# NVlabs/CenterPose

Measured on NVIDIA H100. Metric: images/sec at 512x512 DLA-34 (dla_34 + DCNv2, 7 heads, decode + PnP), higher is better.
Workload: dtype tf32x3

## Files before the change

### centerpose_b200/csrc/common.cuh

```cuda
#pragma once
#include <cuda_runtime.h>
#include <stdint.h>
#include <stdio.h>
#include <string>

#include "../../include/centerpose_b200.h"

namespace cp {

void set_error(const std::string& msg);
int fail(int code, const std::string& msg);
extern thread_local long long g_launch_counter;

#define CP_CUDA_CHECK(expr)                                                              \
  do {                                                                                   \
    cudaError_t _e = (expr);                                                             \
    if (_e != cudaSuccess)                                                               \
      return ::cp::fail(CP_ERR_CUDA, std::string(#expr) + ": " + cudaGetErrorString(_e)); \
  } while (0)

#define CP_LAUNCH_CHECK(what)                                                            \
  do {                                                                                   \
    cudaError_t _e = cudaGetLastError();                                                 \
    if (_e != cudaSuccess)                                                               \
// ... 16 lines not shown
  int srcStride[4];
  int nsrc;
  int B, Hin, Win, Cin;
  int Hout, Wout, Cout, CoutPad;
  int kh, kw, stride, pad;
  int Kpad;
  const float* wgt;
  const float* bias;
  const float* residual;
  int resStride;
  int relu;
  int res_after_relu;
  float* out;
  int outStride;
  int out_nchw;
  const float* offmask;
  int omStride;
  int mask_is_logit;
  int mode;
  const void* wgt_umma;
  float* splitk_ws;
  size_t splitk_ws_floats;
  int fuse_n, fuse_hidden;
  const float* fuse_w[16];
  const float* fuse_b[16];
  float* fuse_out[16];
  int fuse_cout[16];
  int ipm;
  long long wstride, tstride;
  unsigned nchw_per_model;
};
inline int model_ipm(const IgemmParams& p) { return p.ipm > 0 ? p.ipm : p.B; }

int launch_igemm_fp32(const IgemmParams& p, cudaStream_t stream);

int decode_pnp_models(const cp_decode_params* prm, int models, const cp_heads* heads, const double* meta, float* dets,
                      float* poses, int32_t* n_valid, void* workspace, size_t workspace_bytes, void* stream);

struct LaunchInfo {
  int BN = 0;
  int ksplit = 1;
  long long grid = 0;
};

bool conv3_c16_supported(const IgemmParams& p);
int launch_conv3_c16(const IgemmParams& p, cudaStream_t stream);
bool stem_supported(const IgemmParams& p);
// ... 129 lines not shown
```

### centerpose_b200/csrc/conv_tma.cu

```cuda
#include <cuda.h>

#include "common.cuh"
#include "umma_common.cuh"

namespace cp {
namespace {

constexpr int TM_BM = 128;
constexpr int TM_THREADS = 384;
constexpr int TM_THREADS_X3 = 512;

struct TmaConvParams {
  CUtensorMap amap[4];
  int nsrc;
  int srcC[4];
  int B, H, W, Cin, Cout, CoutPad, BN;
  int k;
  int tile_m;
  int Wt, boxh;
  int tiles_per_image;
  long long total_tiles;
  long long m_tiles;
  uint32_t slab_bytes, slab_stride;
  int SA, SB;
  const float* bias;
  const float* residual;
  int resStride, relu, res_after_relu;
  float* out;
  int outStride, out_nchw;
  int round_tf32;
  int cslab;
  int x3;
  int group;
  const unsigned char* wtiles;
  int ksplit, sps;
  float* part;
  int fuse, tph;
  const float* fuse_w[16];
  const float* fuse_b[16];
  float* fuse_out[16];
  int fuse_cout[16];
  int ipm;
  long long wstride, tstride, tiles_per_model;
};

using namespace umma;

struct TmaCtl {
  unsigned long long a_full[4], a_empty[4], a_split[4];
  unsigned long long b_full[8], b_empty[8];
};
static_assert(sizeof(TmaCtl) <= 512, "control block");

struct TileGeo {
  int n_tile, img, g0, r_lo, model;
  long long pos0;
};
template <bool MULTI>
__device__ __forceinline__ TileGeo decode_tile(const TmaConvParams& p, long long ct, int n_tiles) {
  TileGeo g;
  g.n_tile = (int)(ct % n_tiles);
// ... 20 lines not shown

template <bool MULTI>
__device__ __forceinline__ bool tile_position(const TmaConvParams& p, const TileGeo& g, int i, int* n, int* oy, int* ox, int* m) {
  bool valid;
  if (p.k == 3) {
    const int gg = g.g0 + i;
    *oy = gg / p.Wt;
    const int xp = gg - *oy * p.Wt;
    *ox = xp - 1;
    *n = g.img;
    valid = (*oy < p.H) && (xp >= 1) && (xp <= p.W);
  } else {
    const long long pix = g.pos0 + i;
    valid = pix < (MULTI ? (long long)(g.model + 1) * p.ipm : (long long)p.B) * p.H * p.W;
    const long long pp = valid ? pix : 0;
    *ox = (int)(pp % p.W);
    const long long t = pp / p.W;
    *oy = (int)(t % p.H);
    *n = (int)(t / p.H);
  }
  *m = (int)(((size_t)*n * p.H + *oy) * p.W + *ox);
  return valid;
}

template <bool X3, bool FUSE, int BN, bool MULTI>
__global__ void __launch_bounds__(X3 ? TM_THREADS_X3 : TM_THREADS, 1) conv_tma_kernel(const __grid_constant__ TmaConvParams p) {
  extern __shared__ __align__(1024) unsigned char smem[];
  TmaCtl* ctl = reinterpret_cast<TmaCtl*>(smem);
  if (threadIdx.x == 0) griddep_launch_dependents();
  const uint32_t slabs0 = (smem_u32(smem) + 512u + 1023u) & ~1023u;
  const uint32_t rowb = (uint32_t)p.cslab * 4u;
  const uint32_t btile_bytes = (uint32_t)BN * rowb * (X3 ? 2u : 1u);
  const uint32_t a_stage = p.slab_stride * (X3 ? 2u : 1u);
  const uint32_t btiles0 = slabs0 + (uint32_t)p.SA * a_stage;
  const uint32_t drain0 = btiles0 + (uint32_t)p.SB * btile_bytes;

  const int tid = threadIdx.x, warp = tid >> 5, lane = tid & 31;
  const int n_tiles = p.CoutPad / BN;
  const int taps = p.k * p.k;
  const int KS_SPLIT = p.ksplit;
  const int sps = p.sps;
  const int KB = sps * taps;
  const int KB_all = (p.Cin / p.cslab) * taps;
  const long long total_tiles = p.total_tiles;
  const long long tph = FUSE ? p.tph : 1;
  auto tile_at = [&](long long it) { return ((long long)blockIdx.x + (it / tph) * gridDim.x) * tph + (it % tph); };
// ... 28 lines not shown
              cb += p.srcC[src];
              ++src;
            }
            mbar_wait(smem_u32(&ctl->a_empty[stage]), phase ^ 1u);
            const uint32_t bar = smem_u32(&ctl->a_full[stage]);
            mbar_arrive_expect_tx(bar, p.slab_bytes);
            const uint32_t dst = slabs0 + (uint32_t)stage * a_stage;
            if (p.k == 3)
              tma_load_4d(dst, &p.amap[src], s * p.cslab - cb, -1, g.r_lo - 1, g.img, bar);
            else
              tma_load_2d(dst, &p.amap[src], s * p.cslab - cb, (int)g.pos0, bar);
            if (++stage == p.SA) {
              stage = 0;
              phase ^= 1u;
            }
          }
        }
      }
      __syncwarp();
    } else if (warp == 1) {
      if (lane == 0) {
        int stage = 0;
        uint32_t phase = 0;
        for (long long it = 0, tile = tile_at(0); tile < total_tiles; tile = tile_at(++it)) {
          const unsigned char* wsrc;
          if constexpr (MULTI) {
            const TileGeo g = decode_tile<MULTI>(p, tile / KS_SPLIT, n_tiles);
            wsrc = p.wtiles + (size_t)g.model * p.tstride +
                   ((size_t)g.n_tile * KB_all + (size_t)(tile % KS_SPLIT) * KB) * btile_bytes;
          } else {
            const int n_tile = (int)((tile / KS_SPLIT) % n_tiles);
            wsrc = p.wtiles + ((size_t)n_tile * KB_all + (size_t)(tile % KS_SPLIT) * KB) * btile_bytes;
          }
          for (int kb = 0; kb < KB; ++kb) {
            mbar_wait(smem_u32(&ctl->b_empty[stage]), phase ^ 1u);
            const uint32_t bar = smem_u32(&ctl->b_full[stage]);
            mbar_arrive_expect_tx(bar, btile_bytes);
            bulk_g2s(btiles0 + (uint32_t)stage * btile_bytes, wsrc + (size_t)kb * btile_bytes, btile_bytes, bar);
            if (++stage == p.SB) {
              stage = 0;
              phase ^= 1u;
            }
          }
        }
      }
      __syncwarp();
    }
  } else if (X3 && warp >= 12) {
    asm volatile("setmaxnreg.dec.sync.aligned.u32 48;");
    const int st = tid - 384;
    int stage = 0;
    uint32_t phase = 0;
    const uint32_t nchunk = p.slab_bytes >> 4;
    for (long long it = 0, tile = tile_at(0); tile < total_tiles; tile = tile_at(++it)) {
      for (int s = 0; s < sps; ++s) {
        mbar_wait(smem_u32(&ctl->a_full[stage]), phase);
        const uint32_t hi = slabs0 + (uint32_t)stage * a_stage;
        const uint32_t lo = hi + p.slab_stride;
        for (uint32_t c0 = st; c0 < nchunk; c0 += 128 * 4) {
          float4 v[4];
#pragma unroll
// ... 26 lines not shown
    float* dstage = reinterpret_cast<float*>(smem + (drain0 - smem_u32(smem))) + (size_t)c * (DRAIN_STAGE_BYTES / 4);
    const uint32_t bar_a = smem_u32(X3 ? &ctl->a_split[0] : &ctl->a_full[0]);
    const uint32_t bar_a_empty = smem_u32(&ctl->a_empty[0]);
    const uint32_t bar_b_full = smem_u32(&ctl->b_full[0]), bar_b_empty = smem_u32(&ctl->b_empty[0]);
    const uint32_t a_lo_u = p.slab_stride >> 4, b_lo_u = ((uint32_t)BN * rowb) >> 4;
    EpiParams ep;
    ep.bias = p.bias;
    ep.residual = p.residual;
    ep.resStride = p.resStride;
    ep.relu = p.relu;
    ep.res_after_relu = p.res_after_relu;
    ep.round_tf32 = p.round_tf32;
    ep.out = p.out;
    ep.outStride = p.outStride;
    ep.out_nchw = p.out_nchw;
    ep.Cout = p.Cout;
    ep.CoutPad = p.CoutPad;
    ep.H = p.H;
    ep.W = p.W;
    int sa = 0, sb = 0;
    uint32_t pa = 0, pb = 0;
    float acc[BN / 2];
    float sums[X3 ? BN / 2 : 1];
    float acc2[FUSE ? 16 : 1];
#pragma unroll
    for (int j = 0; j < BN / 2; ++j) acc[j] = 0.f;
#pragma unroll
    for (int j = 0; j < (FUSE ? 16 : 1); ++j) acc2[j] = 0.f;
    for (long long it = 0, tile = tile_at(0); tile < total_tiles; tile = tile_at(++it)) {
      const TileGeo g = decode_tile<MULTI>(p, tile / KS_SPLIT, n_tiles);
      const uint32_t row0 = (p.k == 3 ? (uint32_t)(g.g0 - 1 - g.r_lo * p.Wt) : 0u) + (uint32_t)c * 64u;
#pragma unroll
      for (int j = 0; j < (X3 ? BN / 2 : 1); ++j) sums[j] = 0.f;
      const int group = X3 ? p.group : 1;
      const bool overlap = X3 && p.SA > 1;
      int tap = 0;
      auto release_prev = [&]() {
        if (wt == 0) {
          mbar_arrive(bar_b_empty + 8u * (uint32_t)(sb == 0 ? p.SB - 1 : sb - 1));
          if (tap == 0) mbar_arrive(bar_a_empty + 8u * (uint32_t)(sa == 0 ? p.SA - 1 : sa - 1));
        }
      };
      for (int kb0 = 0; kb0 < KB; kb0 += group) {
        const int n_kb = min(group, KB - kb0);
        for (int i = 0; i < n_kb; ++i) {
          if (tap == 0) mbar_wait(bar_a + 8u * (uint32_t)sa, pa);
          const int ky = tap / 3, kx = tap - ky * 3;
          const uint32_t arow = row0 + (p.k == 3 ? (uint32_t)(ky * p.Wt + kx) : 0u);
          mbar_wait(bar_b_full + 8u * (uint32_t)sb, pb);
          const uint64_t da = make_desc(slabs0 + (uint32_t)sa * a_stage + arow * rowb, p.cslab);
          const uint64_t db = make_desc(btiles0 + (uint32_t)sb * btile_bytes, p.cslab);
// ... 12 lines not shown
          }
          if (++tap == taps) {
            tap = 0;
            if (++sa == p.SA) {
              sa = 0;
              pa ^= 1u;
            }
          }
          if (!overlap) {
            wg_wait<0>();
            release_prev();
          }
        }
        wg_wait<0>();
        if (overlap) release_prev();
#pragma unroll
        for (int j = 0; j < (X3 ? BN / 2 : 1); ++j)
          if (X3) sums[j] += acc[X3 ? j : 0];
      }
      if (X3) {
#pragma unroll
        for (int j = 0; j < BN / 2; ++j) acc[j] = 0.f;
      }
      const int r_me = wt >> 1;
      int n, oy, ox, m;
      const bool valid = tile_position<MULTI>(p, g, c * 64 + r_me, &n, &oy, &ox, &m);
      const int col_end = min(p.Cout, (g.n_tile + 1) * BN);
      const int head = FUSE ? g.n_tile / p.tph : 0, part = FUSE ? g.n_tile - head * p.tph : 0;
      const size_t wofs = MULTI ? (size_t)g.model * p.wstride : 0;
      if (MULTI) ep.bias = p.bias + wofs;
      if (FUSE && part == 0) {
#pragma unroll
        for (int j = 0; j < (FUSE ? 16 : 1); ++j) acc2[j] = 0.f;
      }
      auto fn = [&](int r, int cb, float (&v)[16]) {
        if (cb >= BN) return;
        if (!FUSE && KS_SPLIT > 1) {
          const long long mn = tile / KS_SPLIT;
          const int ks = (int)(tile % KS_SPLIT);
          float4* mine = reinterpret_cast<float4*>(p.part) + (((size_t)mn * KS_SPLIT + ks) * (BN >> 2) + (cb >> 2)) * p.tile_m +
                         c * 64 + r;
#pragma unroll
          for (int q = 0; q < 4; ++q) __stcg(mine + (size_t)q * p.tile_m, make_float4(v[4 * q], v[4 * q + 1], v[4 * q + 2], v[4 * q + 3]));
        } else if (FUSE) {
          const float* b1 = p.bias + wofs + (size_t)g.n_tile * BN + cb;
          const float4* w2 = reinterpret_cast<const float4*>(p.fuse_w[head] + wofs) + ((size_t)part * BN + cb) * 4;
#pragma unroll
          for (int q = 0; q < 16; ++q) {
            const float h = fmaxf(v[q] + __ldg(b1 + q), 0.f);
#pragma unroll
            for (int u = 0; u < 4; ++u) {
              const float4 w = __ldg(w2 + q * 4 + u);
              acc2[FUSE ? 4 * u + 0 : 0] = fmaf(h, w.x, acc2[FUSE ? 4 * u + 0 : 0]);
              acc2[FUSE ? 4 * u + 1 : 0] = fmaf(h, w.y, acc2[FUSE ? 4 * u + 1 : 0]);
              acc2[FUSE ? 4 * u + 2 : 0] = fmaf(h, w.z, acc2[FUSE ? 4 * u + 2 : 0]);
              acc2[FUSE ? 4 * u + 3 : 0] = fmaf(h, w.w, acc2[FUSE ? 4 * u + 3 : 0]);
            }
          }
        } else {
          epilogue_row<16>(ep, v, valid, m, n, oy, ox, g.n_tile * BN + cb, col_end);
        }
      };
      if constexpr (X3 && FUSE) {
        const int rg = wt >> 3, hh = (wt >> 2) & 1, og = wt & 3;
        const int fr0 = (wt >> 5) * 16 + ((wt & 31) >> 2), fcq = (wt & 3) * 2;
        const float* b1 = p.bias + wofs + (size_t)g.n_tile * BN;
        const float4* w2 = reinterpret_cast<const float4*>(p.fuse_w[head] + wofs) + (size_t)part * BN * 4 + og;
        auto at = [&](int r, int col) { return r * 32 + ((((col >> 2) ^ r) & 7) << 2) + (col & 3); };
#pragma unroll
        for (int c0 = 0; c0 < BN; c0 += 32) {
#pragma unroll
          for (int j = 0; j < BN / 8; ++j) {
            if (j * 8 >= c0 && j * 8 < c0 + 32) {
              const int col = j * 8 - c0 + fcq;
              const float bx = __ldg(b1 + c0 + col), by = __ldg(b1 + c0 + col + 1);
              dstage[at(fr0, col)] = fmaxf(sums[X3 ? 4 * j : 0] + bx, 0.f);
              dstage[at(fr0, col + 1)] = fmaxf(sums[X3 ? 4 * j + 1 : 0] + by, 0.f);
              dstage[at(fr0 + 8, col)] = fmaxf(sums[X3 ? 4 * j + 2 : 0] + bx, 0.f);
              dstage[at(fr0 + 8, col + 1)] = fmaxf(sums[X3 ? 4 * j + 3 : 0] + by, 0.f);
            }
          }
          wg_bar_sync(1 + c);
#pragma unroll
          for (int m4 = 0; m4 < 4; ++m4) {
            const int k0 = 16 * hh + 4 * m4;
            float4 hv[4];
#pragma unroll
            for (int i = 0; i < 4; ++i) hv[i] = *reinterpret_cast<const float4*>(dstage + at(rg + 16 * i, k0));
#pragma unroll
            for (int kk = 0; kk < 4; ++kk) {
              const float4 w = __ldg(w2 + (size_t)(c0 + k0 + kk) * 4);
#pragma unroll
              for (int i = 0; i < 4; ++i) {
                const float h = kk == 0 ? hv[i].x : kk == 1 ? hv[i].y : kk == 2 ? hv[i].z : hv[i].w;
                acc2[FUSE ? 4 * i + 0 : 0] = fmaf(h, w.x, acc2[FUSE ? 4 * i + 0 : 0]);
                acc2[FUSE ? 4 * i + 1 : 0] = fmaf(h, w.y, acc2[FUSE ? 4 * i + 1 : 0]);
                acc2[FUSE ? 4 * i + 2 : 0] = fmaf(h, w.z, acc2[FUSE ? 4 * i + 2 : 0]);
                acc2[FUSE ? 4 * i + 3 : 0] = fmaf(h, w.w, acc2[FUSE ? 4 * i + 3 : 0]);
              }
            }
          }
          wg_bar_sync(1 + c);
        }
        if (part == p.tph - 1) {
#pragma unroll
          for (int j = 0; j < 16; ++j) acc2[FUSE ? j : 0] += __shfl_xor_sync(0xffffffffu, acc2[FUSE ? j : 0], 4);
          if (hh == 0) {
            const int co = p.fuse_cout[head];
            const size_t plane = (size_t)p.H * p.W;
#pragma unroll
            for (int i = 0; i < 4; ++i) {
              int n1, oy1, ox1, m1;
              if (!tile_position<MULTI>(p, g, c * 64 + rg + 16 * i, &n1, &oy1, &ox1, &m1)) continue;
              float* o = p.fuse_out[head] + ((size_t)n1 * co * p.H + oy1) * p.W + ox1;
#pragma unroll
              for (int u = 0; u < 4; ++u)
                if (4 * og + u < co) o[(4 * og + u) * plane] = acc2[FUSE ? 4 * i + u : 0] + __ldg(p.fuse_b[head] + wofs + 4 * og + u);
            }
          }
        }
        continue;
      }
      if constexpr (X3)
        drain_rows<BN>(sums, dstage, wt, 1 + c, fn);
      else
        drain_rows<BN>(acc, dstage, wt, 1 + c, fn);
      if (FUSE && part == p.tph - 1) {
#pragma unroll
        for (int j = 0; j < (FUSE ? 16 : 1); ++j) acc2[j] += __shfl_xor_sync(0xffffffffu, acc2[j], 1);
        if ((wt & 1) == 0 && valid) {
          const int co = p.fuse_cout[head];
          float* o = p.fuse_out[head] + ((size_t)n * co * p.H + oy) * p.W + ox;
          const size_t plane = (size_t)p.H * p.W;
#pragma unroll
          for (int j = 0; j < 16; ++j)
            if (j < co) o[j * plane] = acc2[FUSE ? j : 0] + __ldg(p.fuse_b[head] + wofs + j);
        }
      }
    }
  }
}

__global__ void pack_tma_weight_kernel(const float* __restrict__ src, int ld, int Cin, int taps, int Cout, int BN, int n_tiles,
                                       int round_tf32, int x3, int cslab, unsigned char* __restrict__ dst) {
  const int KB = (Cin / cslab) * taps;
  const int cpr = cslab / 4;
  const size_t rowb = (size_t)cslab * 4;
  const size_t total = (size_t)n_tiles * KB * BN * cpr;
  for (size_t i = blockIdx.x * (size_t)blockDim.x + threadIdx.x; i < total; i += (size_t)gridDim.x * blockDim.x) {
    const int q = i % cpr;
    size_t t = i / cpr;
    const int nr = t % BN;
    t /= BN;
    const int kb = t % KB;
    const int nt = t / KB;
    const int n = nt * BN + nr;
    const int slab = kb / taps, tap = kb - slab * taps;
    float v[4];
#pragma unroll
    for (int j = 0; j < 4; ++j) {
      const int k = tap * Cin + slab * cslab + q * 4 + j;
// ... 143 lines not shown
      cuuint32_t box[4] = {(cuuint32_t)cs, (cuuint32_t)Wt, (cuuint32_t)boxh, 1};
      cuuint32_t es[4] = {1, 1, 1, 1};
      r = enc(&maps[s], CU_TENSOR_MAP_DATA_TYPE_FLOAT32, 4, (void*)p.src[s], dims, strides, box, es,
              CU_TENSOR_MAP_INTERLEAVE_NONE, swz, CU_TENSOR_MAP_L2_PROMOTION_L2_256B,
              CU_TENSOR_MAP_FLOAT_OOB_FILL_NONE);
    } else {
      cuuint64_t dims[2] = {(cuuint64_t)p.srcC[s], (cuuint64_t)Bmax * p.Hin * p.Win};
      cuuint64_t strides[1] = {(cuuint64_t)p.srcStride[s] * 4};
      cuuint32_t box[2] = {(cuuint32_t)cs, (cuuint32_t)TM_BM};
      cuuint32_t es[2] = {1, 1};
      r = enc(&maps[s], CU_TENSOR_MAP_DATA_TYPE_FLOAT32, 2, (void*)p.src[s], dims, strides, box, es,
              CU_TENSOR_MAP_INTERLEAVE_NONE, swz, CU_TENSOR_MAP_L2_PROMOTION_L2_256B,
              CU_TENSOR_MAP_FLOAT_OOB_FILL_NONE);
    }
    if (r != CUDA_SUCCESS) return fail(CP_ERR_CUDA, "cuTensorMapEncodeTiled failed with code " + std::to_string((int)r));
  }
  return CP_OK;
}

template <bool X3, bool FUSE, bool MULTI>
static int launch_conv_tma_kernel(const TmaConvParams& q, const cudaLaunchConfig_t& cfg0) {
  void (*kern)(TmaConvParams) = nullptr;
  switch (q.BN) {
    case 16: kern = conv_tma_kernel<X3, FUSE, 16, MULTI>; break;
    case 32: kern = conv_tma_kernel<X3, FUSE, 32, MULTI>; break;
    case 64: kern = conv_tma_kernel<X3, FUSE, 64, MULTI>; break;
    case 128: kern = conv_tma_kernel<X3, FUSE, 128, MULTI>; break;
    default: return fail(CP_ERR_INVALID, "conv_tma: unsupported N tile");
  }
  static PerDevice<bool, 4> configured;
  const int slot = q.BN == 128 ? 3 : (q.BN == 64 ? 2 : (q.BN == 32 ? 1 : 0));
  if (!configured.here(slot)) {
    CP_CUDA_CHECK(cudaFuncSetAttribute(kern, cudaFuncAttributeMaxDynamicSharedMemorySize, 227 * 1024));
    configured.here(slot) = true;
  }
  cudaLaunchConfig_t cfg = cfg0;
  cudaLaunchAttribute attr[1];
  attr[0].id = cudaLaunchAttributeProgrammaticStreamSerialization;
  attr[0].val.programmaticStreamSerializationAllowed = 1;
  cfg.attrs = attr;
  cfg.numAttrs = g_pdl ? 1 : 0;
  CP_CUDA_CHECK(cudaLaunchKernelEx(&cfg, kern, q));
  CP_LAUNCH_CHECK("conv_tma_kernel");
  return CP_OK;
}

int launch_conv_tma(const IgemmParams& p, const void* maps, const ConvKernel& k, cudaStream_t stream, LaunchInfo* info) {
  if (!p.wgt_umma) return fail(CP_ERR_INVALID, "conv_tma: weight tiles missing");
  if (p.B % model_ipm(p)) return fail(CP_ERR_INVALID, "conv_tma: batch is not a whole number of models");
  const bool x3 = k.x3;
  TmaConvParams q;
  memset(&q, 0, sizeof(q));
// ... 24 lines not shown
    q.slab_bytes = (uint32_t)q.boxh * q.Wt * (uint32_t)q.cslab * 4u;
  } else {
    q.tiles_per_image = 0;
    q.tiles_per_model = ((long long)q.ipm * p.Hin * p.Win + q.tile_m - 1) / q.tile_m;
    m_tiles = (size_t)q.tiles_per_model * (p.B / q.ipm);
    q.slab_bytes = (uint32_t)q.tile_m * (uint32_t)q.cslab * 4u;
  }
  q.slab_stride = (q.slab_bytes + 1023u) & ~1023u;
  const uint32_t btile = (uint32_t)q.BN * (uint32_t)q.cslab * 4u * (x3 ? 2u : 1u);
  const uint32_t a_stage = q.slab_stride * (x3 ? 2u : 1u);
  size_t smem = 0;
  if (int rc = tma_smem_layout(a_stage, btile, q.k, &q.SA, &q.SB, &smem)) return rc;
  q.bias = p.bias;
  q.residual = p.residual;
  q.resStride = p.resStride;
  q.relu = p.relu;
  q.res_after_relu = p.res_after_relu;
  q.out = p.out;
  q.outStride = p.outStride;
  q.out_nchw = p.out_nchw;
  q.round_tf32 = k.round_out;
  q.wtiles = (const unsigned char*)p.wgt_umma;
  if (p.fuse_n > 0) {
    if (p.fuse_hidden % q.BN || p.CoutPad != p.fuse_n * p.fuse_hidden || !p.relu || p.residual || (x3 && q.BN != 128))
      return fail(CP_ERR_INVALID, "conv_tma: fused 1x1 needs relu, no residual and head_conv a multiple of the N tile");
    q.fuse = 1;
    q.tph = p.fuse_hidden / q.BN;
    for (int h = 0; h < p.fuse_n; ++h) {
      q.fuse_w[h] = p.fuse_w[h];
      q.fuse_b[h] = p.fuse_b[h];
      q.fuse_out[h] = p.fuse_out[h];
      q.fuse_cout[h] = p.fuse_cout[h];
    }
  }
  q.m_tiles = (long long)m_tiles;
  q.part = p.splitk_ws;
  const long long mn = (long long)m_tiles * (p.CoutPad / q.BN);
  const int nslab = q.Cin / q.cslab;
  int num_sms = 0;
  if (int rc = device_sm_count(&num_sms)) return rc;
  q.ksplit = x3 && !q.fuse ? splitk_factor(mn, nslab, num_sms, (size_t)q.tile_m * q.BN, p.splitk_ws_floats) : 1;
  q.sps = nslab / q.ksplit;
  q.total_tiles = mn * q.ksplit;
  if (q.total_tiles >= (1ll << 31)) return fail(CP_ERR_INVALID, "conv_tma: too many tiles");
  cudaLaunchConfig_t cfg{};
  cfg.gridDim = dim3((unsigned)(q.total_tiles < num_sms ? q.total_tiles : num_sms));
  cfg.blockDim = dim3(x3 ? TM_THREADS_X3 : TM_THREADS);
  cfg.dynamicSmemBytes = smem;
  cfg.stream = stream;
  const bool multi = p.B > q.ipm;
  int rc;
  if (multi)
// ... 22 lines not shown
```

### centerpose_b200/csrc/plan.cu

```cuda
#include <stdlib.h>
#include <string.h>

#include <map>
#include <memory>
#include <set>
#include <string>
#include <vector>

#include "arena_pack.h"
#include "common.cuh"

namespace cp {

thread_local std::string g_last_error;
void set_error(const std::string& msg) { g_last_error = msg; }
thread_local long long g_launch_counter = 0;
thread_local int g_pdl = 0;

int fail(int code, const std::string& msg) {
  g_last_error = msg;
  return code;
}

namespace {
// ... 74 lines not shown

}
}

using namespace cp;

struct cp_plan {
  cp_config cfg;
  std::vector<std::string> head_names;
  int B = 0, H = 0, W = 0;
  std::vector<Op> ops;
  std::vector<PackJob> jobs;
  float* act = nullptr;
  size_t act_floats = 0;
  float* wts = nullptr;
  size_t w_floats = 0;
  std::vector<Act> head_bufs;
  bool loaded = false;
  int launches = 0;
  void* decode_ws = nullptr;
  size_t decode_ws_bytes = 0;
  double* gn_stats = nullptr;
  bool no_dcn_tma = false;
  unsigned char* umma_wts = nullptr;
  size_t umma_bytes = 0;
  float* splitk_ws = nullptr;
  int models = 1;
  std::vector<char> model_loaded;
  unsigned ext_per_model = 0;
  bool reuse = false;
  std::vector<ArenaAlloc> bufs;
  std::vector<size_t> buf_off;
};

namespace cp {
namespace {

struct Builder {
  cp_plan* P;
  size_t act_cur = 0, w_cur = 0;
  int B;

  size_t walloc(size_t n) {
    size_t o = w_cur;
    w_cur += (n + 63) / 64 * 64;
    return o;
// ... 458 lines not shown
  p.residual = op.has_res ? P->act + op.res.off : nullptr;
  p.resStride = op.res.stride;
  p.relu = op.relu;
  p.res_after_relu = op.res_after_relu;
  if (op.out_head >= 0) {
    p.out = head_out ? head_out[op.out_head] : nullptr;
    p.out_nchw = 1;
    p.outStride = 0;
  } else {
    p.out = P->act + op.out.off;
    p.outStride = op.out.stride;
  }
  if (op.mode == IGEMM_DCN) {
    p.offmask = P->act + op.om.off;
    p.omStride = op.om.stride;
    p.mask_is_logit = 1;
  }
  p.mode = op.mode;
  if (op.fuse_heads) {
    p.fuse_n = (int)op.head_children.size();
    p.fuse_hidden = P->cfg.head_conv;
    for (int i = 0; i < p.fuse_n; ++i) {
      const Op& ch = P->ops[op.head_children[i]];
      p.fuse_w[i] = P->wts + ch.w_off;
      p.fuse_b[i] = P->wts + ch.b_off;
      p.fuse_out[i] = head_out ? head_out[ch.out_head] : nullptr;
      p.fuse_cout[i] = ch.Cout;
    }
  }
}

void plan_params(const cp_plan* P, const Op& op, IgemmParams* p) {
  static const float* const no_ext[4] = {};
  igemm_params(P, op, P->B, no_ext, nullptr, p);
}

void select_kernels(cp_plan* P) {
  const ConvPolicy pol{true, !P->no_dcn_tma, true, true};
  static const float residual_present = 0.f;
  P->umma_bytes = 0;
  for (auto& op : P->ops) {
    if (op.type != OP_IGEMM) continue;
    IgemmParams p;
    plan_params(P, op, &p);
    if (op.has_res) p.residual = &residual_present;
    op.kernel = select_conv_kernel(p, P->cfg.precision, pol);
    op.tile_off = P->umma_bytes;
    P->umma_bytes += (op.kernel.wbytes + 1023) / 1024 * 1024;
  }
  const int head_conv = P->cfg.head_conv;
  for (auto& op : P->ops) {
    if (op.head_children.empty() || op.kernel.family != CP_FAM_CONV_TMA) continue;
    const int bn = op.kernel.BN;
    bool ok = op.relu && !op.has_res && (head_conv % bn == 0) && (int)op.head_children.size() <= 16 &&
              op.CoutPad == (int)op.head_children.size() * head_conv && (!op.kernel.x3 || bn == 128);
    for (int ci : op.head_children) {
      const Op& ch = P->ops[ci];
      ok = ok && ch.CoutPad == 16 && ch.w_ld == 16 && ch.Cin == head_conv && ch.out_head >= 0 && !ch.relu && !ch.has_res;
    }
    if (!ok) continue;
    op.fuse_heads = true;
    for (int ci : op.head_children) P->ops[ci].fused_away = true;
  }
}

template <class F>
void for_each_act(cp_plan* P, Op& op, F f) {
  if (op.fused_away) return;
  switch (op.type) {
    case OP_IGEMM:
      for (int s = 0; s < op.nsrc; ++s) f(op.src[s]);
      if (op.has_res) f(op.res);
      if (op.mode == IGEMM_DCN) f(op.om);
      if (op.out_head >= 0) f(P->head_bufs[op.out_head]);
      else if (!op.fuse_heads) f(op.out);
      if (op.fuse_heads)
        for (int c : op.head_children) f(P->head_bufs[P->ops[c].out_head]);
      return;
    case OP_MAXPOOL:
    case OP_MAXPOOL3:
    case OP_UPADD:
// ... 105 lines not shown
  if (cfg->height % 32 || cfg->width % 32 || cfg->height <= 0 || cfg->width <= 0)
    return fail(CP_ERR_INVALID, "cp_plan_create: height/width must be positive multiples of 32");
  if (cfg->max_batch <= 0 || cfg->num_heads <= 0 || cfg->num_heads > CP_MAX_HEADS)
    return fail(CP_ERR_INVALID, "cp_plan_create: bad batch / head count");
  if (cfg->head_conv <= 0 || cfg->head_conv % 64)
    return fail(CP_ERR_INVALID, "cp_plan_create: head_conv must be a positive multiple of 64");
  if (cfg->arch == CP_ARCH_DLAV1_34 && cfg->head_conv != 256)
    return fail(CP_ERR_INVALID, "cp_plan_create: dlav1 GroupNorm path needs head_conv == 256");
  P->cfg = *cfg;
  for (int i = 0; i < cfg->num_heads; ++i) {
    if (!cfg->head_names[i] || cfg->head_channels[i] <= 0 || cfg->head_channels[i] > 16)
      return fail(CP_ERR_INVALID, "cp_plan_create: head channels must be in 1..16");
    P->head_names.push_back(cfg->head_names[i]);
  }
  for (int i = 0; i < cfg->num_heads; ++i) P->cfg.head_names[i] = P->head_names[i].c_str();
  P->B = cfg->max_batch;
  P->models = num_models;
  P->ext_per_model = (flags & CP_PLAN_MULTI_TRACK) ? kMultiTrackInputs : 0u;
  P->reuse = (flags & CP_PLAN_REUSE_ACTIVATIONS) != 0;
  P->model_loaded.assign(num_models, 0);
  P->H = cfg->height;
  P->W = cfg->width;
  if (const char* e = getenv("CP_NO_DCN_TMA")) P->no_dcn_tma = atoi(e) != 0;
  if (int rc = build_graph(P)) return rc;
  select_kernels(P);
  layout_arena(P);
  return CP_OK;
}

static void plan_memory(const cp_plan* P, cp_memory_info* m) {
  const bool splitk = P->cfg.precision == CP_PREC_TF32X3 || P->cfg.precision == CP_PREC_TF32;
  m->activation_bytes = (int64_t)(P->act_floats * sizeof(float));
  m->weight_bytes = (int64_t)(P->w_floats * P->models * sizeof(float));
  m->tile_bytes = (int64_t)(P->umma_bytes * P->models);
  m->workspace_bytes = (int64_t)(sizeof(double) * gn_workspace_doubles(P->B * P->models) +
                                 (splitk ? kSplitkWsFloats * sizeof(float) : 0));
}

static int create_plan(const cp_config* cfg, int32_t num_models, uint32_t flags, cp_plan** out) {
  std::unique_ptr<cp_plan> P(new cp_plan());
  if (int rc = plan_layout(P.get(), cfg, num_models, flags)) return rc;
  struct DeviceGuard {
    int prev = -1;
    ~DeviceGuard() {
      if (prev >= 0) cudaSetDevice(prev);
    }
// ... 547 lines not shown
```

### centerpose_b200/csrc/umma_common.cuh

```cuda
#pragma once
#include <cuda.h>
#include <cuda_runtime.h>
#include <stdint.h>
#include <stdio.h>

namespace cp {
namespace umma {

__device__ __forceinline__ uint32_t smem_u32(const void* p) { return (uint32_t)__cvta_generic_to_shared(p); }

__device__ __forceinline__ void mbar_init(uint32_t bar, uint32_t count) {
  asm volatile("mbarrier.init.shared::cta.b64 [%0], %1;" ::"r"(bar), "r"(count));
}
__device__ __forceinline__ void mbar_arrive(uint32_t bar) {
  asm volatile("mbarrier.arrive.shared::cta.b64 _, [%0];" ::"r"(bar) : "memory");
}
__device__ __forceinline__ void mbar_arrive_expect_tx(uint32_t bar, uint32_t bytes) {
  asm volatile("mbarrier.arrive.expect_tx.shared::cta.b64 _, [%0], %1;" ::"r"(bar), "r"(bytes) : "memory");
}
__device__ __forceinline__ bool mbar_try_wait(uint32_t bar, uint32_t parity) {
  uint32_t ok;
  asm volatile(
      "{\n\t.reg .pred p;\n\tmbarrier.try_wait.parity.shared::cta.b64 p, [%1], %2;\n\tselp.b32 %0, 1, 0, p;\n\t}"
      : "=r"(ok)
// ... 151 lines not shown
  }
  if (X3) {
#pragma unroll
    for (int ks = 0; ks < KS; ++ks) wgmma_tf32<BN>(acc, da + 2u * ks, db + 2u * ks, 1u);
  }
  wg_commit();
}
template <int BN, bool X3, bool BF16, int KS>
__device__ __forceinline__ void mma_kblock(float (&acc)[BN / 2], uint64_t da, uint64_t db, uint32_t a_lo, uint32_t b_lo,
                                           bool fresh) {
  mma_kblock_issue<BN, X3, BF16, KS>(acc, da, db, a_lo, b_lo, fresh);
  wg_wait<0>();
}

__device__ __forceinline__ float tf32_round(float x) {
  return __uint_as_float((__float_as_uint(x) + 0x1000u) & 0xffffe000u);
}
__device__ __forceinline__ void ldsm_x4(uint32_t (&r)[4], uint32_t addr) {
  asm volatile("ldmatrix.sync.aligned.m8n8.x4.shared.b16 {%0, %1, %2, %3}, [%4];"
               : "=r"(r[0]), "=r"(r[1]), "=r"(r[2]), "=r"(r[3])
               : "r"(addr));
}

template <int BN, int KS>
__device__ __forceinline__ void mma_kblock_x3(float (&acc)[BN / 2], uint32_t a_tile, int wt, uint64_t db, uint32_t b_lo,
                                              bool fresh) {
  const uint32_t lane = (uint32_t)wt & 31u;
  const uint32_t row = (uint32_t)(wt >> 5) * 16u + (lane & 7u) + ((lane >> 3) & 1u) * 8u;
  const uint32_t a_row = a_tile + row * (32u * KS);
  const uint32_t x = ((lane >> 4) << 4) ^ ((a_row >> 3) & (KS == 4 ? 0x70u : 0x30u));
  uint32_t hi[KS][4], lo[KS][4];
#pragma unroll
  for (int ks = 0; ks < KS; ++ks) {
    ldsm_x4(hi[ks], a_row + (((uint32_t)ks << 5) ^ x));
#pragma unroll
    for (int j = 0; j < 4; ++j) {
      const float v = __uint_as_float(hi[ks][j]);
      const float h = tf32_round(v);
      lo[ks][j] = __float_as_uint(tf32_round(v - h));
      hi[ks][j] = __float_as_uint(h);
    }
  }
  wg_fence();
#pragma unroll
  for (int ks = 0; ks < KS; ++ks) {
    wgmma_tf32_rs<BN>(acc, lo[ks], db + 2u * ks, (fresh && ks == 0) ? 0u : 1u);
    wgmma_tf32_rs<BN>(acc, hi[ks], db + b_lo + 2u * ks, 1u);
  }
#pragma unroll
  for (int ks = 0; ks < KS; ++ks) wgmma_tf32_rs<BN>(acc, hi[ks], db + 2u * ks, 1u);
  wg_commit();
  wg_wait<0>();
#pragma unroll
  for (int ks = 0; ks < KS; ++ks)
#pragma unroll
    for (int j = 0; j < 4; ++j) asm volatile("" : "+r"(hi[ks][j]), "+r"(lo[ks][j]));
}

__device__ __forceinline__ uint32_t pack_bf16x2(float a, float b) {
  uint32_t r;
  asm("cvt.rn.bf16x2.f32 %0, %1, %2;" : "=r"(r) : "f"(b), "f"(a));
  return r;
}
__device__ __forceinline__ void st_shared_v4(uint32_t addr, uint32_t a, uint32_t b, uint32_t c, uint32_t d) {
  asm volatile("st.shared.v4.b32 [%0], {%1, %2, %3, %4};" ::"r"(addr), "r"(a), "r"(b), "r"(c), "r"(d) : "memory");
}
__device__ __forceinline__ void st_shared_v4f(uint32_t addr, float a, float b, float c, float d) {
  asm volatile("st.shared.v4.f32 [%0], {%1, %2, %3, %4};" ::"r"(addr), "f"(a), "f"(b), "f"(c), "f"(d) : "memory");
}
__device__ __forceinline__ float4 ld_shared_v4f(uint32_t addr) {
  float4 v;
  asm volatile("ld.shared.v4.f32 {%0,%1,%2,%3}, [%4];" : "=f"(v.x), "=f"(v.y), "=f"(v.z), "=f"(v.w) : "r"(addr) : "memory");
  return v;
}
// ... 142 lines not shown
```

Baseline: 739.1.

## Run fused head 1x1 second GEMM on wgmma tensor cores with TMA-loaded weight tiles

The fused head path previously computed the second 1x1 conv (hidden to up to 16 outputs) with scalar FMAs per thread, reading weights through __ldg and, for x3, staging activations in shared memory with barriers. It now feeds the ReLU'd accumulator registers directly as wgmma register A operands via lane shuffles, and loads the pre-tiled head weights through the existing B-tile bulk-copy pipeline as an extra stage per tile. The x3 split-precision issue is factored into a shared helper. This removes the CUDA-core FMA and shared-memory staging cost, but adds an extra pipeline stage, shuffle overhead and a restriction to BN of at least 64.

```diff
diff --git a/centerpose_b200/csrc/common.cuh b/centerpose_b200/csrc/common.cuh
--- a/centerpose_b200/csrc/common.cuh
+++ b/centerpose_b200/csrc/common.cuh
@@ -62,7 +62,7 @@
   float* splitk_ws;
   size_t splitk_ws_floats;
   int fuse_n, fuse_hidden;
-  const float* fuse_w[16];
+  const void* fuse_tiles[16];
   const float* fuse_b[16];
   float* fuse_out[16];
   int fuse_cout[16];
diff --git a/centerpose_b200/csrc/conv_tma.cu b/centerpose_b200/csrc/conv_tma.cu
--- a/centerpose_b200/csrc/conv_tma.cu
+++ b/centerpose_b200/csrc/conv_tma.cu
@@ -36,7 +36,7 @@
   int ksplit, sps;
   float* part;
   int fuse, tph;
-  const float* fuse_w[16];
+  const unsigned char* fuse_tiles[16];
   const float* fuse_b[16];
   float* fuse_out[16];
   int fuse_cout[16];
@@ -103,6 +103,11 @@
   *m = (int)(((size_t)*n * p.H + *oy) * p.W + *ox);
   return valid;
 }
+
+constexpr uint32_t kFuseKBlockBytes = 16u * 32u * 4u;
+constexpr int kFuseKBlocks = 2;
+template <bool FUSE>
+__device__ __forceinline__ int b_stages_per_tile(int KB) { return KB + (FUSE ? 1 : 0); }
 
 template <bool X3, bool FUSE, int BN, bool MULTI>
 __global__ void __launch_bounds__(X3 ? TM_THREADS_X3 : TM_THREADS, 1) conv_tma_kernel(const __grid_constant__ TmaConvParams p) {
@@ -177,21 +182,31 @@
       if (lane == 0) {
         int stage = 0;
         uint32_t phase = 0;
+        const uint32_t fuse_bytes = (uint32_t)(BN / 32) * kFuseKBlockBytes * (X3 ? 2u : 1u);
         for (long long it = 0, tile = tile_at(0); tile < total_tiles; tile = tile_at(++it)) {
           const unsigned char* wsrc;
+          int n_tile;
+          size_t tofs = 0;
           if constexpr (MULTI) {
             const TileGeo g = decode_tile<MULTI>(p, tile / KS_SPLIT, n_tiles);
-            wsrc = p.wtiles + (size_t)g.model * p.tstride +
-                   ((size_t)g.n_tile * KB_all + (size_t)(tile % KS_SPLIT) * KB) * btile_bytes;
+            n_tile = g.n_tile;
+            tofs = (size_t)g.model * p.tstride;
           } else {
-            const int n_tile = (int)((tile / KS_SPLIT) % n_tiles);
-            wsrc = p.wtiles + ((size_t)n_tile * KB_all + (size_t)(tile % KS_SPLIT) * KB) * btile_bytes;
-          }
-          for (int kb = 0; kb < KB; ++kb) {
+            n_tile = (int)((tile / KS_SPLIT) % n_tiles);
+          }
+          wsrc = p.wtiles + tofs + ((size_t)n_tile * KB_all + (size_t)(tile % KS_SPLIT) * KB) * btile_bytes;
+          const unsigned char* fsrc = nullptr;
+          if (FUSE) {
+            const int head = n_tile / p.tph;
+            fsrc = p.fuse_tiles[head] + tofs + (size_t)(n_tile - head * p.tph) * fuse_bytes;
+          }
+          for (int kb = 0; kb < b_stages_per_tile<FUSE>(KB); ++kb) {
+            const bool fz = FUSE && kb == KB;
+            const uint32_t bytes = fz ? fuse_bytes : btile_bytes;
             mbar_wait(smem_u32(&ctl->b_empty[stage]), phase ^ 1u);
             const uint32_t bar = smem_u32(&ctl->b_full[stage]);
-            mbar_arrive_expect_tx(bar, btile_bytes);
-            bulk_g2s(btiles0 + (uint32_t)stage * btile_bytes, wsrc + (size_t)kb * btile_bytes, btile_bytes, bar);
+            mbar_arrive_expect_tx(bar, bytes);
+            bulk_g2s(btiles0 + (uint32_t)stage * btile_bytes, fz ? fsrc : wsrc + (size_t)kb * btile_bytes, bytes, bar);
             if (++stage == p.SB) {
               stage = 0;
               phase ^= 1u;
@@ -264,11 +279,9 @@
     uint32_t pa = 0, pb = 0;
     float acc[BN / 2];
     float sums[X3 ? BN / 2 : 1];
-    float acc2[FUSE ? 16 : 1];
+    float acc1[FUSE && !X3 ? 8 : 1], sums2[FUSE && X3 ? 8 : 1];
 #pragma unroll
     for (int j = 0; j < BN / 2; ++j) acc[j] = 0.f;
-#pragma unroll
-    for (int j = 0; j < (FUSE ? 16 : 1); ++j) acc2[j] = 0.f;
     for (long long it = 0, tile = tile_at(0); tile < total_tiles; tile = tile_at(++it)) {
       const TileGeo g = decode_tile<MULTI>(p, tile / KS_SPLIT, n_tiles);
       const uint32_t row0 = (p.k == 3 ? (uint32_t)(g.g0 - 1 - g.r_lo * p.Wt) : 0u) + (uint32_t)c * 64u;
@@ -327,121 +340,139 @@
 #pragma unroll
         for (int j = 0; j < BN / 2; ++j) acc[j] = 0.f;
       }
+      if constexpr (FUSE) {
+        const int head = g.n_tile / p.tph, part = g.n_tile - head * p.tph;
+        const size_t wofs = MULTI ? (size_t)g.model * p.wstride : 0;
+        const float* b1 = p.bias + wofs + (size_t)g.n_tile * BN;
+        const int q = lane & 3, src1 = ((q & 1) << 1) | (q >> 1);
+        const bool up = (q >> 1) != 0, odd = (q & 1) != 0;
+        if (X3 && part == 0) {
+#pragma unroll
+          for (int j = 0; j < 8; ++j) sums2[X3 ? j : 0] = 0.f;
+        }
+        for (int s = KB; s < b_stages_per_tile<FUSE>(KB); ++s) {
+          mbar_wait(bar_b_full + 8u * (uint32_t)sb, pb);
+          const uint64_t dw = make_desc(btiles0 + (uint32_t)sb * btile_bytes, 32);
+#pragma unroll
+          for (int kb0 = 0; kb0 < BN / 32; kb0 += kFuseKBlocks) {
+            uint32_t a[kFuseKBlocks][4][4];
+#pragma unroll
+            for (int b = 0; b < kFuseKBlocks; ++b)
+#pragma unroll
+              for (int ks = 0; ks < 4; ++ks) {
+                const int j = 4 * (kb0 + b) + ks;
+                const float bx = __ldg(b1 + 8 * j + 2 * q), by = __ldg(b1 + 8 * j + 2 * q + 1);
+                float e[4];
+#pragma unroll
+                for (int u = 0; u < 4; ++u) {
+                  const float v = (X3 ? sums[X3 ? 4 * j + u : 0] : acc[4 * j + u]) + ((u & 1) ? by : bx);
+                  e[u] = fmaxf(v, 0.f);
+                  if (p.round_tf32) e[u] = tf32_round(e[u]);
+                }
+#pragma unroll
+                for (int i = 0; i < 2; ++i) {
+                  const float r1 = __shfl_sync(0xffffffffu, up ? e[2 * i + 1] : e[2 * i], src1, 4);
+                  const float r2 = __shfl_sync(0xffffffffu, up ? e[2 * i] : e[2 * i + 1], src1 ^ 2, 4);
+                  a[b][ks][i] = __float_as_uint(odd ? r2 : r1);
+                  a[b][ks][2 + i] = __float_as_uint(odd ? r1 : r2);
+                }
+              }
+            if constexpr (X3) {
+              uint32_t lo[kFuseKBlocks][4][4];
+              float acc2[kFuseKBlocks][8];
+#pragma unroll
+              for (int b = 0; b < kFuseKBlocks; ++b)
+#pragma unroll
+                for (int ks = 0; ks < 4; ++ks)
+#pragma unroll
+                  for (int u = 0; u < 4; ++u) {
+                    const float v = __uint_as_float(a[b][ks][u]);
+                    const float h = tf32_round(v);
+                    lo[b][ks][u] = __float_as_uint(tf32_round(v - h));
+                    a[b][ks][u] = __float_as_uint(h);
+                  }
+              mma_x3_rs_issue<16, 4, kFuseKBlocks>(acc2, a, lo, dw + (uint32_t)kb0 * (2u * kFuseKBlockBytes >> 4),
+                                                   kFuseKBlockBytes >> 4, true, 2u * kFuseKBlockBytes >> 4);
+              wg_wait<0>();
+#pragma unroll
+              for (int b = 0; b < kFuseKBlocks; ++b) {
+#pragma unroll
+                for (int ks = 0; ks < 4; ++ks)
+#pragma unroll
+                  for (int u = 0; u < 4; ++u) asm volatile("" : "+r"(a[b][ks][u]), "+r"(lo[b][ks][u]));
+#pragma unroll
+                for (int u = 0; u < 8; ++u) sums2[X3 ? u : 0] += acc2[b][u];
+              }
+            } else {
+              wg_fence();
+#pragma unroll
+              for (int b = 0; b < kFuseKBlocks; ++b)
+#pragma unroll
+                for (int ks = 0; ks < 4; ++ks)
+                  wgmma_tf32_rs<16>(acc1, a[b][ks], dw + (uint32_t)(kb0 + b) * (kFuseKBlockBytes >> 4) + 2u * ks,
+                                    (part == 0 && kb0 + b == 0 && ks == 0) ? 0u : 1u);
+              wg_commit();
+              wg_wait<0>();
+#pragma unroll
+              for (int b = 0; b < kFuseKBlocks; ++b)
+#pragma unroll
+                for (int ks = 0; ks < 4; ++ks)
+#pragma unroll
+                  for (int u = 0; u < 4; ++u) asm volatile("" : "+r"(a[b][ks][u]));
+            }
+          }
+          if (wt == 0) mbar_arrive(bar_b_empty + 8u * (uint32_t)sb);
+          if (++sb == p.SB) {
+            sb = 0;
+            pb ^= 1u;
+          }
+        }
+        if (part == p.tph - 1) {
+          const int co = p.fuse_cout[head];
+          const float* b2 = p.fuse_b[head] + wofs;
+          const size_t plane = (size_t)p.H * p.W;
+#pragma unroll
+          for (int i = 0; i < 2; ++i) {
+            int n1, oy1, ox1, m1;
+            if (!tile_position<MULTI>(p, g, c * 64 + (wt >> 5) * 16 + (lane >> 2) + 8 * i, &n1, &oy1, &ox1, &m1)) continue;
+            float* o = p.fuse_out[head] + ((size_t)n1 * co * p.H + oy1) * p.W + ox1;
+#pragma unroll
+            for (int j = 0; j < 2; ++j)
+#pragma unroll
+              for (int u = 0; u < 2; ++u) {
+                const int col = 8 * j + 2 * q + u;
+                if (col >= co) continue;
+                float v = (X3 ? sums2[X3 ? 4 * j + 2 * i + u : 0] : acc1[X3 ? 0 : 4 * j + 2 * i + u]) + __ldg(b2 + col);
+                if (p.round_tf32) v = tf32_round(v);
+                o[col * plane] = v;
+              }
+          }
+        }
+        continue;
+      }
       const int r_me = wt >> 1;
       int n, oy, ox, m;
       const bool valid = tile_position<MULTI>(p, g, c * 64 + r_me, &n, &oy, &ox, &m);
       const int col_end = min(p.Cout, (g.n_tile + 1) * BN);
-      const int head = FUSE ? g.n_tile / p.tph : 0, part = FUSE ? g.n_tile - head * p.tph : 0;
       const size_t wofs = MULTI ? (size_t)g.model * p.wstride : 0;
       if (MULTI) ep.bias = p.bias + wofs;
-      if (FUSE && part == 0) {
-#pragma unroll
-        for (int j = 0; j < (FUSE ? 16 : 1); ++j) acc2[j] = 0.f;
-      }
       auto fn = [&](int r, int cb, float (&v)[16]) {
         if (cb >= BN) return;
-        if (!FUSE && KS_SPLIT > 1) {
+        if (KS_SPLIT > 1) {
           const long long mn = tile / KS_SPLIT;
           const int ks = (int)(tile % KS_SPLIT);
           float4* mine = reinterpret_cast<float4*>(p.part) + (((size_t)mn * KS_SPLIT + ks) * (BN >> 2) + (cb >> 2)) * p.tile_m +
                          c * 64 + r;
 #pragma unroll
           for (int q = 0; q < 4; ++q) __stcg(mine + (size_t)q * p.tile_m, make_float4(v[4 * q], v[4 * q + 1], v[4 * q + 2], v[4 * q + 3]));
-        } else if (FUSE) {
-          const float* b1 = p.bias + wofs + (size_t)g.n_tile * BN + cb;
-          const float4* w2 = reinterpret_cast<const float4*>(p.fuse_w[head] + wofs) + ((size_t)part * BN + cb) * 4;
-#pragma unroll
-          for (int q = 0; q < 16; ++q) {
-            const float h = fmaxf(v[q] + __ldg(b1 + q), 0.f);
-#pragma unroll
-            for (int u = 0; u < 4; ++u) {
-              const float4 w = __ldg(w2 + q * 4 + u);
-              acc2[FUSE ? 4 * u + 0 : 0] = fmaf(h, w.x, acc2[FUSE ? 4 * u + 0 : 0]);
-              acc2[FUSE ? 4 * u + 1 : 0] = fmaf(h, w.y, acc2[FUSE ? 4 * u + 1 : 0]);
-              acc2[FUSE ? 4 * u + 2 : 0] = fmaf(h, w.z, acc2[FUSE ? 4 * u + 2 : 0]);
-              acc2[FUSE ? 4 * u + 3 : 0] = fmaf(h, w.w, acc2[FUSE ? 4 * u + 3 : 0]);
-            }
-          }
         } else {
           epilogue_row<16>(ep, v, valid, m, n, oy, ox, g.n_tile * BN + cb, col_end);
         }
       };
-      if constexpr (X3 && FUSE) {
-        const int rg = wt >> 3, hh = (wt >> 2) & 1, og = wt & 3;
-        const int fr0 = (wt >> 5) * 16 + ((wt & 31) >> 2), fcq = (wt & 3) * 2;
-        const float* b1 = p.bias + wofs + (size_t)g.n_tile * BN;
-        const float4* w2 = reinterpret_cast<const float4*>(p.fuse_w[head] + wofs) + (size_t)part * BN * 4 + og;
-        auto at = [&](int r, int col) { return r * 32 + ((((col >> 2) ^ r) & 7) << 2) + (col & 3); };
-#pragma unroll
-        for (int c0 = 0; c0 < BN; c0 += 32) {
-#pragma unroll
-          for (int j = 0; j < BN / 8; ++j) {
-            if (j * 8 >= c0 && j * 8 < c0 + 32) {
-              const int col = j * 8 - c0 + fcq;
-              const float bx = __ldg(b1 + c0 + col), by = __ldg(b1 + c0 + col + 1);
-              dstage[at(fr0, col)] = fmaxf(sums[X3 ? 4 * j : 0] + bx, 0.f);
-              dstage[at(fr0, col + 1)] = fmaxf(sums[X3 ? 4 * j + 1 : 0] + by, 0.f);
-              dstage[at(fr0 + 8, col)] = fmaxf(sums[X3 ? 4 * j + 2 : 0] + bx, 0.f);
-              dstage[at(fr0 + 8, col + 1)] = fmaxf(sums[X3 ? 4 * j + 3 : 0] + by, 0.f);
-            }
-          }
-          wg_bar_sync(1 + c);
-#pragma unroll
-          for (int m4 = 0; m4 < 4; ++m4) {
-            const int k0 = 16 * hh + 4 * m4;
-            float4 hv[4];
-#pragma unroll
-            for (int i = 0; i < 4; ++i) hv[i] = *reinterpret_cast<const float4*>(dstage + at(rg + 16 * i, k0));
-#pragma unroll
-            for (int kk = 0; kk < 4; ++kk) {
-              const float4 w = __ldg(w2 + (size_t)(c0 + k0 + kk) * 4);
-#pragma unroll
-              for (int i = 0; i < 4; ++i) {
-                const float h = kk == 0 ? hv[i].x : kk == 1 ? hv[i].y : kk == 2 ? hv[i].z : hv[i].w;
-                acc2[FUSE ? 4 * i + 0 : 0] = fmaf(h, w.x, acc2[FUSE ? 4 * i + 0 : 0]);
-                acc2[FUSE ? 4 * i + 1 : 0] = fmaf(h, w.y, acc2[FUSE ? 4 * i + 1 : 0]);
-                acc2[FUSE ? 4 * i + 2 : 0] = fmaf(h, w.z, acc2[FUSE ? 4 * i + 2 : 0]);
-                acc2[FUSE ? 4 * i + 3 : 0] = fmaf(h, w.w, acc2[FUSE ? 4 * i + 3 : 0]);
-              }
-            }
-          }
-          wg_bar_sync(1 + c);
-        }
-        if (part == p.tph - 1) {
-#pragma unroll
-          for (int j = 0; j < 16; ++j) acc2[FUSE ? j : 0] += __shfl_xor_sync(0xffffffffu, acc2[FUSE ? j : 0], 4);
-          if (hh == 0) {
-            const int co = p.fuse_cout[head];
-            const size_t plane = (size_t)p.H * p.W;
-#pragma unroll
-            for (int i = 0; i < 4; ++i) {
-              int n1, oy1, ox1, m1;
-              if (!tile_position<MULTI>(p, g, c * 64 + rg + 16 * i, &n1, &oy1, &ox1, &m1)) continue;
-              float* o = p.fuse_out[head] + ((size_t)n1 * co * p.H + oy1) * p.W + ox1;
-#pragma unroll
-              for (int u = 0; u < 4; ++u)
-                if (4 * og + u < co) o[(4 * og + u) * plane] = acc2[FUSE ? 4 * i + u : 0] + __ldg(p.fuse_b[head] + wofs + 4 * og + u);
-            }
-          }
-        }
-        continue;
-      }
       if constexpr (X3)
         drain_rows<BN>(sums, dstage, wt, 1 + c, fn);
       else
         drain_rows<BN>(acc, dstage, wt, 1 + c, fn);
-      if (FUSE && part == p.tph - 1) {
-#pragma unroll
-        for (int j = 0; j < (FUSE ? 16 : 1); ++j) acc2[j] += __shfl_xor_sync(0xffffffffu, acc2[j], 1);
-        if ((wt & 1) == 0 && valid) {
-          const int co = p.fuse_cout[head];
-          float* o = p.fuse_out[head] + ((size_t)n * co * p.H + oy) * p.W + ox;
-          const size_t plane = (size_t)p.H * p.W;
-#pragma unroll
-          for (int j = 0; j < 16; ++j)
-            if (j < co) o[j * plane] = acc2[FUSE ? j : 0] + __ldg(p.fuse_b[head] + wofs + j);
-        }
-      }
     }
   }
 }
@@ -631,12 +662,13 @@
 static int launch_conv_tma_kernel(const TmaConvParams& q, const cudaLaunchConfig_t& cfg0) {
   void (*kern)(TmaConvParams) = nullptr;
   switch (q.BN) {
-    case 16: kern = conv_tma_kernel<X3, FUSE, 16, MULTI>; break;
-    case 32: kern = conv_tma_kernel<X3, FUSE, 32, MULTI>; break;
+    case 16: if constexpr (!FUSE) kern = conv_tma_kernel<X3, FUSE, 16, MULTI>; break;
+    case 32: if constexpr (!FUSE) kern = conv_tma_kernel<X3, FUSE, 32, MULTI>; break;
     case 64: kern = conv_tma_kernel<X3, FUSE, 64, MULTI>; break;
     case 128: kern = conv_tma_kernel<X3, FUSE, 128, MULTI>; break;
-    default: return fail(CP_ERR_INVALID, "conv_tma: unsupported N tile");
-  }
+    default: break;
+  }
+  if (!kern) return fail(CP_ERR_INVALID, "conv_tma: unsupported N tile");
   static PerDevice<bool, 4> configured;
   const int slot = q.BN == 128 ? 3 : (q.BN == 64 ? 2 : (q.BN == 32 ? 1 : 0));
   if (!configured.here(slot)) {
@@ -707,12 +739,14 @@
   q.round_tf32 = k.round_out;
   q.wtiles = (const unsigned char*)p.wgt_umma;
   if (p.fuse_n > 0) {
-    if (p.fuse_hidden % q.BN || p.CoutPad != p.fuse_n * p.fuse_hidden || !p.relu || p.residual || (x3 && q.BN != 128))
+    if (p.fuse_hidden % q.BN || p.CoutPad != p.fuse_n * p.fuse_hidden || !p.relu || p.residual || (x3 && q.BN != 128) ||
+        q.BN < 64)
       return fail(CP_ERR_INVALID, "conv_tma: fused 1x1 needs relu, no residual and head_conv a multiple of the N tile");
     q.fuse = 1;
     q.tph = p.fuse_hidden / q.BN;
     for (int h = 0; h < p.fuse_n; ++h) {
-      q.fuse_w[h] = p.fuse_w[h];
+      if (!p.fuse_tiles[h]) return fail(CP_ERR_INVALID, "conv_tma: fused 1x1 weight tiles missing");
+      q.fuse_tiles[h] = (const unsigned char*)p.fuse_tiles[h];
       q.fuse_b[h] = p.fuse_b[h];
       q.fuse_out[h] = p.fuse_out[h];
       q.fuse_cout[h] = p.fuse_cout[h];
diff --git a/centerpose_b200/csrc/plan.cu b/centerpose_b200/csrc/plan.cu
--- a/centerpose_b200/csrc/plan.cu
+++ b/centerpose_b200/csrc/plan.cu
@@ -120,6 +120,7 @@
   size_t decode_ws_bytes = 0;
   double* gn_stats = nullptr;
   bool no_dcn_tma = false;
+  bool no_fuse_heads = false;
   unsigned char* umma_wts = nullptr;
   size_t umma_bytes = 0;
   float* splitk_ws = nullptr;
@@ -624,7 +625,7 @@
     p.fuse_hidden = P->cfg.head_conv;
     for (int i = 0; i < p.fuse_n; ++i) {
       const Op& ch = P->ops[op.head_children[i]];
-      p.fuse_w[i] = P->wts + ch.w_off;
+      p.fuse_tiles[i] = P->umma_wts ? P->umma_wts + ch.tile_off : nullptr;
       p.fuse_b[i] = P->wts + ch.b_off;
       p.fuse_out[i] = head_out ? head_out[ch.out_head] : nullptr;
       p.fuse_cout[i] = ch.Cout;
@@ -652,13 +653,15 @@
   }
   const int head_conv = P->cfg.head_conv;
   for (auto& op : P->ops) {
-    if (op.head_children.empty() || op.kernel.family != CP_FAM_CONV_TMA) continue;
+    if (P->no_fuse_heads || op.head_children.empty() || op.kernel.family != CP_FAM_CONV_TMA) continue;
     const int bn = op.kernel.BN;
-    bool ok = op.relu && !op.has_res && (head_conv % bn == 0) && (int)op.head_children.size() <= 16 &&
+    bool ok = op.relu && !op.has_res && (head_conv % bn == 0) && bn >= 64 && (int)op.head_children.size() <= 16 &&
               op.CoutPad == (int)op.head_children.size() * head_conv && (!op.kernel.x3 || bn == 128);
     for (int ci : op.head_children) {
       const Op& ch = P->ops[ci];
       ok = ok && ch.CoutPad == 16 && ch.w_ld == 16 && ch.Cin == head_conv && ch.out_head >= 0 && !ch.relu && !ch.has_res;
+      ok = ok && ch.kernel.family == CP_FAM_CONV_TMA && ch.kernel.x3 == op.kernel.x3 && ch.kernel.BN == 16 &&
+           ch.kernel.cslab == 32 && ch.kernel.round_out == op.kernel.round_out;
     }
     if (!ok) continue;
     op.fuse_heads = true;
@@ -810,6 +813,7 @@
   P->H = cfg->height;
   P->W = cfg->width;
   if (const char* e = getenv("CP_NO_DCN_TMA")) P->no_dcn_tma = atoi(e) != 0;
+  if (const char* e = getenv("CP_NO_FUSE_HEADS")) P->no_fuse_heads = atoi(e) != 0;
   if (int rc = build_graph(P)) return rc;
   select_kernels(P);
   layout_arena(P);
diff --git a/centerpose_b200/csrc/umma_common.cuh b/centerpose_b200/csrc/umma_common.cuh
--- a/centerpose_b200/csrc/umma_common.cuh
+++ b/centerpose_b200/csrc/umma_common.cuh
@@ -197,6 +197,25 @@
                : "r"(addr));
 }
 
+template <int BN, int KS, int NB = 1>
+__device__ __forceinline__ void mma_x3_rs_issue(float (&acc)[NB][BN / 2], const uint32_t (&hi)[NB][KS][4],
+                                                const uint32_t (&lo)[NB][KS][4], uint64_t db, uint32_t b_lo, bool fresh,
+                                                uint32_t b_step = 0) {
+  wg_fence();
+#pragma unroll
+  for (int ks = 0; ks < KS; ++ks) {
+#pragma unroll
+    for (int b = 0; b < NB; ++b) wgmma_tf32_rs<BN>(acc[b], lo[b][ks], db + b * b_step + 2u * ks, (fresh && ks == 0) ? 0u : 1u);
+#pragma unroll
+    for (int b = 0; b < NB; ++b) wgmma_tf32_rs<BN>(acc[b], hi[b][ks], db + b * b_step + b_lo + 2u * ks, 1u);
+  }
+#pragma unroll
+  for (int ks = 0; ks < KS; ++ks)
+#pragma unroll
+    for (int b = 0; b < NB; ++b) wgmma_tf32_rs<BN>(acc[b], hi[b][ks], db + b * b_step + 2u * ks, 1u);
+  wg_commit();
+}
+
 template <int BN, int KS>
 __device__ __forceinline__ void mma_kblock_x3(float (&acc)[BN / 2], uint32_t a_tile, int wt, uint64_t db, uint32_t b_lo,
                                               bool fresh) {
@@ -216,15 +235,9 @@
       hi[ks][j] = __float_as_uint(h);
     }
   }
-  wg_fence();
-#pragma unroll
-  for (int ks = 0; ks < KS; ++ks) {
-    wgmma_tf32_rs<BN>(acc, lo[ks], db + 2u * ks, (fresh && ks == 0) ? 0u : 1u);
-    wgmma_tf32_rs<BN>(acc, hi[ks], db + b_lo + 2u * ks, 1u);
-  }
-#pragma unroll
-  for (int ks = 0; ks < KS; ++ks) wgmma_tf32_rs<BN>(acc, hi[ks], db + 2u * ks, 1u);
-  wg_commit();
+  using One = uint32_t[1][KS][4];
+  mma_x3_rs_issue<BN, KS>(reinterpret_cast<float(&)[1][BN / 2]>(acc), reinterpret_cast<One&>(hi), reinterpret_cast<One&>(lo),
+                          db, b_lo, fresh);
   wg_wait<0>();
 #pragma unroll
   for (int ks = 0; ks < KS; ++ks)
```

After: 761.2 (median of 6 runs). +3.0%, better.
